# AWehenkel/Graphical-Normalizing-Flows

Measured on AMD Instinct MI355X. Metric: samples/sec (fwd+log|detJ|+bwd) MNIST d=784 Monotonic-DAG, higher is better.
Workload: dtype f32; 1 GPU; cfg4: MNIST d=784, MonotonicNormalizer[50,50,50] cond 30 S=20 + DAGConditioner(MNISTCNN->30, prior_A_kernel=2, hot_encoding=False, Gumbel gate T=1), b_size=100 per GPU; step = fwd+logdet+NLL+bwd+allreduce+Adam; global_batch=100, parallelism=dp1

## Files before the change

graphical-normalizing-flows_amd/gnf_hip/csrc/gnf_mnistcnn.h:

```cpp
#pragma once
#include "gnf_common.h"

namespace {

constexpr int IMG = 28, C1 = 26, C2 = 24, PO = 12, NCH = 16;
constexpr int ROWE = 36, ESZ = IMG * ROWE;
constexpr int ROW = 40, CH = C1 * ROW;
constexpr int ROWD = 40, CHD = 28 * ROWD + 16;
constexpr int CS = 676;
constexpr int NPOOL = NCH * PO * PO;
constexpr int FWD_WAVES = 8, BWD_WAVES = 8;
constexpr int PROW = NCH * 144 + NCH * 16 + NCH;

static_assert(CH % 32 == 16 && CHD % 32 == 16, "channel strides must sit 16 banks apart");

__device__ __forceinline__ f32x2 pk_v12(f32x2 a, f32x2 b) {
  f32x2 r;
  asm("v_pk_add_f32 %0, %1, %2 op_sel:[1,0] op_sel_hi:[1,0] neg_hi:[1,0]" : "=v"(r) : "v"(a), "v"(b));
  return r;
}
__device__ __forceinline__ void wino_in(const f32x2 (&lo)[4], const f32x2 (&hi)[4], float (&v)[16]) {
  f32x2 tl[4], th[4];
  tl[0] = lo[0] - lo[2]; th[0] = hi[0] - hi[2];
  tl[1] = lo[1] + lo[2]; th[1] = hi[1] + hi[2];
  tl[2] = lo[2] - lo[1]; th[2] = hi[2] - hi[1];
  tl[3] = lo[1] - lo[3]; th[3] = hi[1] - hi[3];
#pragma unroll
  for (int rr = 0; rr < 4; ++rr) {
    const f32x2 v03 = tl[rr] - th[rr], v12 = pk_v12(tl[rr], th[rr]);
    v[4 * rr + 0] = v03.x; v[4 * rr + 1] = v12.x; v[4 * rr + 2] = v12.y; v[4 * rr + 3] = v03.y;
  }
}

__device__ __forceinline__ float dpp_xor1(float v) {
  return __int_as_float(__builtin_amdgcn_update_dpp(0, __float_as_int(v), 0xB1, 0xF, 0xF, false));
}
__device__ __forceinline__ float dpp_xor8(float v) {
  return __int_as_float(__builtin_amdgcn_update_dpp(0, __float_as_int(v), 0x128, 0xF, 0xF, false));
}

struct CnnArgs {
  const float* e; const float* W1; const float* b1; const float* W2; const float* b2;
  float* pooled; unsigned char* arg;
  const float* gp; const unsigned char* argin; float* ge; float* part;
  int64_t n;
  const int32_t* plan; float* gec; int dplan;
};

template <int NU, int CHS>
__device__ __forceinline__ void conv1_units(const float* e_rd, float* a1_wr, int u0, const float* w1p, const f32x4& b1v,
                                            int q, int j, int lane) {
  u0 = __builtin_amdgcn_readfirstlane(u0);
  asm volatile("" : "+s"(u0));
  f32x16 acc[NU];
  float ev[NU][9], w1a[9];
#pragma unroll
  for (int tap = 0; tap < 9; ++tap) w1a[tap] = w1p[16 * tap];
#pragma unroll
  for (int k = 0; k < NU; ++k) {
    const int pos = 64 * (u0 + k) + lane;
    const int pc = pos < C1 * C1 ? pos : 0;
    const float* pe = e_rd + pc + 2 * (int)(__umul24((unsigned)pc, 2521u) >> 16);
#pragma unroll
    for (int tap = 0; tap < 9; ++tap) ev[k][tap] = pe[(tap / 3) * IMG + tap % 3];
#pragma unroll
    for (int v = 0; v < 16; ++v) acc[k][v] = b1v[v & 3];
  }
  __builtin_amdgcn_sched_barrier(0);
#pragma unroll
  for (int tap = 0; tap < 9; ++tap)
#pragma unroll
    for (int k = 0; k < NU; ++k) acc[k] = __builtin_amdgcn_mfma_f32_16x16x1f32(w1a[tap], ev[k][tap], acc[k], 0, 0, 0);
  __builtin_amdgcn_sched_barrier(0);
#pragma unroll
  for (int k = 0; k < NU; ++k)
#pragma unroll
    for (int b = 0; b < 4; ++b) {
      const int pos = 64 * (u0 + k) + 16 * b + j;
      if (pos < C1 * C1) {
        float* pa = a1_wr + 4 * q * CHS + pos + 2 * (int)(__umul24((unsigned)pos, 2521u) >> 16);
#pragma unroll
        for (int r = 0; r < 4; ++r) pa[r * CHS] = relu1(acc[k][4 * b + r]);
      }
    }
}
template <int CHS>
__device__ __forceinline__ void conv1_offsets(int u, int q, int j, int lane, unsigned (&po)[3]) {
  static_assert(CHS >= 26 * IMG + 8, "the dummy stores of off-grid positions land at 26 IMG + (0..7) of the channel");
  const int pos = 64 * u + lane, pc = pos < C1 * C1 ? pos : 0;
  unsigned w[4];
#pragma unroll
  for (int b = 0; b < 4; ++b) {
    const int p = 64 * u + 16 * b + j;
    w[b] = (unsigned)(4 * q * CHS + (p < C1 * C1 ? p + 2 * (p / C1) : 26 * IMG + (j & 7)));
  }
  po[0] = (unsigned)(pc + 2 * (pc / C1)) | (w[0] << 16);
  po[1] = w[1] | (w[2] << 16);
  po[2] = w[3];
}
template <int NU, int CHS>
__device__ __forceinline__ void conv1_units_pre(const float* e_rd, float* a1_wr, const unsigned (&po)[3][3], const float* w1p,
                                                const f32x4& b1v) {
  f32x16 acc[NU];
  float ev[NU][9], w1a[9];
#pragma unroll
  for (int tap = 0; tap < 9; ++tap) w1a[tap] = w1p[16 * tap];
#pragma unroll
  for (int k = 0; k < NU; ++k) {
    const float* pe = e_rd + (po[k][0] & 0xffffu);
#pragma unroll
    for (int tap = 0; tap < 9; ++tap) ev[k][tap] = pe[(tap / 3) * IMG + tap % 3];
#pragma unroll
    for (int v = 0; v < 16; ++v) acc[k][v] = b1v[v & 3];
  }
  __builtin_amdgcn_sched_barrier(0);
#pragma unroll
  for (int tap = 0; tap < 9; ++tap)
#pragma unroll
    for (int k = 0; k < NU; ++k) acc[k] = __builtin_amdgcn_mfma_f32_16x16x1f32(w1a[tap], ev[k][tap], acc[k], 0, 0, 0);
  __builtin_amdgcn_sched_barrier(0);
#pragma unroll
  for (int k = 0; k < NU; ++k) {
    const unsigned off[4] = {po[k][0] >> 16, po[k][1] & 0xffffu, po[k][1] >> 16, po[k][2]};
#pragma unroll
    for (int b = 0; b < 4; ++b) {
      float* pa = a1_wr + off[b];
#pragma unroll
// ... 38 lines not shown
```

graphical-normalizing-flows_amd/gnf_hip/csrc/gnf_mnistcnn.hip:

```cpp
#include "gnf_mnistcnn.h"

namespace {

#ifdef GNF_CNN_TIMING
#define TSTAMP(k) do { const long long t__ = __builtin_readcyclecounter(); tacc[k] += t__ - tlast; tlast = t__; } while (0)
#else
#define TSTAMP(k)
#endif

constexpr int NG4 = 11;
constexpr int USZ = 16 * 4 * 64;
constexpr int ROWB = 28, CHB = 730, A1B = NCH * CHB;
constexpr int ESZB = IMG * IMG;
constexpr int DCS = 648, DPAD = 576, DSZW = NCH * DCS;
static_assert(ROWB == IMG, "the de gather indexes the T planes with the pixel index");
static_assert(CHB >= 25 * ROWB + C1 && CHB % 4 == 2, "a1 channel stride");
static_assert(DCS % 64 == 8 && DCS >= DPAD + 64, "dY2 channel slots");
__device__ __forceinline__ int dslot(int o) { return (o & 3) + 4 * (o >> 3) + 8 * ((o >> 2) & 1); }

#ifndef GNF_BWD_C1U
#define GNF_BWD_C1U {0, 0, 0, 4, 1, 1, 2, 3}
#endif
__device__ constexpr int C1U[8] = GNF_BWD_C1U;
__device__ constexpr int C1PRO[8] = {2, 2, 2, 1, 1, 1, 1, 1};
constexpr int c1sum(const int (&a)[8]) { int s = 0; for (int i = 0; i < 8; ++i) s += a[i]; return s; }
constexpr int NU1 = (C1 * C1 + 63) / 64;
static_assert(c1sum(C1U) == NU1 && c1sum(C1PRO) == NU1, "conv1 units");

__device__ __forceinline__ void conv1_run(const float* e_rd, float* a1_wr, int u0, int nu, const float* w1a,
                                          const f32x4& b1v, int q, int j, int lane) {
  if (nu == 4) {
    conv1_units<2, CHB>(e_rd, a1_wr, u0, w1a, b1v, q, j, lane);
    conv1_units<2, CHB>(e_rd, a1_wr, u0 + 2, w1a, b1v, q, j, lane);
  } else if (nu == 3) conv1_units<3, CHB>(e_rd, a1_wr, u0, w1a, b1v, q, j, lane);
  else if (nu == 2) conv1_units<2, CHB>(e_rd, a1_wr, u0, w1a, b1v, q, j, lane);
  else if (nu == 1) conv1_units<1, CHB>(e_rd, a1_wr, u0, w1a, b1v, q, j, lane);
}

template <int HY>
__device__ __forceinline__ void dw2_phase(const float* av, const float* dz, f32x4 (&dU)[8]) {
  f32x4 zw[2];
  f32x2 dl[2][3], dh[2][3];
  auto load = [&](int st, int b) {
    const int tyl = st / 3, k = st - 3 * tyl;
    zw[b] = *reinterpret_cast<const f32x4*>(dz + 48 * tyl + 16 * k);
#pragma unroll
// ... 4 lines not shown
  };
  load(0, 0);
#pragma unroll
  for (int st = 0; st < 9; ++st) {
    const int b = st & 1;
    f32x2 tal, tah, tbl, tbh;
    float za[2], zb[2];
    if (HY == 0) {
      tal = dl[b][0] - dl[b][2]; tah = dh[b][0] - dh[b][2]; tbl = dl[b][1] + dl[b][2]; tbh = dh[b][1] + dh[b][2];
      za[0] = zw[b][0]; za[1] = zw[b][1]; zb[0] = zw[b][0] + zw[b][2]; zb[1] = zw[b][1] + zw[b][3];
    } else {
      tal = dl[b][1] - dl[b][0]; tah = dh[b][1] - dh[b][0]; tbl = dl[b][0] - dl[b][2]; tbh = dh[b][0] - dh[b][2];
      za[0] = zw[b][0] - zw[b][2]; za[1] = zw[b][1] - zw[b][3]; zb[0] = zw[b][2]; zb[1] = zw[b][3];
    }
    float vv[8], zz[8];
    {
      const f32x2 a03 = tal - tah, a12 = pk_v12(tal, tah), b03 = tbl - tbh, b12 = pk_v12(tbl, tbh);
      vv[0] = a03.x; vv[1] = a12.x; vv[2] = a12.y; vv[3] = a03.y;
      vv[4] = b03.x; vv[5] = b12.x; vv[6] = b12.y; vv[7] = b03.y;
    }
    zz[0] = za[0]; zz[1] = za[0] + za[1]; zz[2] = za[0] - za[1]; zz[3] = za[1];
    zz[4] = zb[0]; zz[5] = zb[0] + zb[1]; zz[6] = zb[0] - zb[1]; zz[7] = zb[1];
    if (st + 1 < 9) load(st + 1, b ^ 1);
    __builtin_amdgcn_sched_barrier(0);
#pragma unroll
    for (int xi = 0; xi < 8; ++xi) dU[xi] = mfma(zz[xi], vv[xi], dU[xi]);
    __builtin_amdgcn_sched_barrier(0);
  }
}

constexpr int KC = GNF_DAG_PLAN_KC;
template <bool SP>
__device__ __forceinline__ void cnn_bwd_body(const CnnArgs& a, float* smem) {
#ifdef GNF_CNN_TIMING
  long long tacc[8] = {0, 0, 0, 0, 0, 0, 0, 0};
  long long tlast = __builtin_readcyclecounter();
#endif
  float* e_s = smem;
  float* a1_s = smem + 2 * ESZB;
  float* d_s = a1_s + 2 * A1B;
  float* u_s = d_s + DSZW;
  unsigned* cnt_s = reinterpret_cast<unsigned*>(u_s + USZ);
  float* w1_s = u_s + USZ + 4;
  unsigned* gmt_s = reinterpret_cast<unsigned*>(w1_s + 9 * NCH);
  const int tid = threadIdx.x, lane = tid & 63, q = lane >> 4, j = lane & 15;
  const int wave = __builtin_amdgcn_readfirstlane(tid >> 6);
  constexpr int NW = BWD_WAVES, NT = 64 * BWD_WAVES;
  static_assert(((2 * ESZB) % 4 == 0) && ((2 * A1B) % 4 == 0) && (DSZW % 4 == 0), "d_s / u_s must be 16-B aligned");

  if (tid < 9 * NCH) w1_s[tid] = a.W1[(tid & 15) * 9 + (tid >> 4)];
  const float* w1a = w1_s + j;
  f32x4 b1v;
#pragma unroll
  for (int r = 0; r < 4; ++r) b1v[r] = a.b1[4 * q + r];
  float w1t[4];
#pragma unroll
  for (int r = 0; r < 4; ++r) w1t[r] = j < 9 ? a.W1[(4 * q + r) * 9 + j] : 0.f;

  if (wave < 4) {
    const int g = wave;
    const float* w = a.W2 + ((4 * q + g) * NCH + j) * 9;
    double gw[4][3];
#pragma unroll
    for (int c = 0; c < 3; ++c) {
      const double w0 = w[8 - c], w1 = w[5 - c], w2 = w[2 - c];
      gw[0][c] = w0; gw[1][c] = 0.5 * (w0 + w1 + w2); gw[2][c] = 0.5 * (w0 - w1 + w2); gw[3][c] = w2;
    }
#pragma unroll
    for (int r = 0; r < 4; ++r) {
      f32x4 u;
      u[0] = (float)gw[r][0];
      u[1] = (float)(0.5 * (gw[r][0] + gw[r][1] + gw[r][2]));
      u[2] = (float)(0.5 * (gw[r][0] - gw[r][1] + gw[r][2]));
      u[3] = (float)gw[r][2];
      *reinterpret_cast<f32x4*>(u_s + ((g * 4 + r) * 64 + lane) * 4) = u;
    }
  }

  const int hy = wave >> 2, wq = wave & 3;
  f32x4 dU[8];
#pragma unroll
  for (int xi = 0; xi < 8; ++xi) dU[xi] = f32x4{0.f, 0.f, 0.f, 0.f};
  f32x2 gW1p[2][10];
#pragma unroll
  for (int h = 0; h < 2; ++h)
#pragma unroll
    for (int k = 0; k < 10; ++k) gW1p[h][k] = f32x2{0.f, 0.f};
  float gb2 = 0.f;
  unsigned aprev = 0;

  for (int i = tid; i < DSZW; i += NT) d_s[i] = 0.f;
  for (int i = tid; i < 2 * A1B; i += NT) a1_s[i] = 0.f;
  if (tid == 0) *cnt_s = 0u;
  const int16_t* const pcols = SP ? reinterpret_cast<const int16_t*>(a.plan + a.dplan) : nullptr;
  if (SP) {
    for (int i = tid; i < a.dplan; i += NT) gmt_s[i] = 0u;
    __syncthreads();
    for (int t = tid; t < a.dplan * KC; t += NT) {
      const int jj = pcols[t];
      if (jj >= 0) {
        const int y = jj / IMG, x = jj - y * IMG;
        unsigned m = 0u;
#pragma unroll
        for (int ky = 0; ky < 3; ++ky)
#pragma unroll
          for (int kx = 0; kx < 3; ++kx) {
            const int py = y - ky, px = x - kx;
            if ((unsigned)py < (unsigned)C1 && (unsigned)px < (unsigned)C1) m |= 1u << ((13 * (py >> 1) + (px >> 1)) >> 4);
          }
        atomicOr(&gmt_s[t / KC], m);
      }
    }
  }

  constexpr int EPT = (IMG * IMG + NT - 1) / NT, WPT = (PO * PO + 31) / 32;
  float epre[EPT], gpre[WPT];
  unsigned apre[WPT];
  auto rsrc_of = [&](const void* base, int64_t im, int bytes) {
    return make_rsrc(static_cast<const char*>(base) + im * bytes, im < a.n ? bytes : 0);
  };
  const int vo_e = tid * 4, vo_g = ((tid >> 5) * (PO * PO) + (tid & 31)) * 4, vo_a = (tid >> 5) * (PO * PO) + (tid & 31);
  auto prefetch_e = [&](int64_t im) {
    const rsrc_t rs = rsrc_of(a.e, im, IMG * IMG * 4);
#pragma unroll
    for (int k = 0; k < EPT; ++k) epre[k] = __builtin_bit_cast(float, __builtin_amdgcn_raw_buffer_load_b32(rs, vo_e + k * NT * 4, 0, 0));
// ... 60 lines not shown
        const int y = (int)(__umul24((unsigned)ic, 2341u) >> 16);
        const float* tp = Tp + ic;
        float t[9];
#pragma unroll
        for (int tap = 0; tap < 9; ++tap) t[tap] = tp[tap * CHB - (tap / 3) * IMG - tap % 3];
        float s = 0.f;
#pragma unroll
        for (int ky = 0; ky < 3; ++ky) {
          const float r3 = (t[3 * ky] + t[3 * ky + 1]) + t[3 * ky + 2];
          s += (unsigned)(y - ky) < (unsigned)C1 ? r3 : 0.f;
        }
        __builtin_amdgcn_raw_buffer_store_b32(__builtin_bit_cast(unsigned, s), rs, i * 4, 0, 0);
      }
    }
  };

  auto de_cols = [&](int64_t im, int cj, const float* Tp) {
    const rsrc_t rs = rsrc_of(a.gec, im, KC * 4);
    const int ic = cj >= 0 ? cj : 0;
    const int y = (int)(__umul24((unsigned)ic, 2341u) >> 16);
    const float* tp = Tp + ic;
    float t[9];
#pragma unroll
    for (int tap = 0; tap < 9; ++tap) t[tap] = tp[tap * CHB - (tap / 3) * IMG - tap % 3];
    float sum = 0.f;
#pragma unroll
    for (int ky = 0; ky < 3; ++ky) {
      const float r3 = (t[3 * ky] + t[3 * ky + 1]) + t[3 * ky + 2];
      sum += (unsigned)(y - ky) < (unsigned)C1 ? r3 : 0.f;
    }
    __builtin_amdgcn_raw_buffer_store_b32(__builtin_bit_cast(unsigned, sum), rs, cj >= 0 && lane < KC ? lane * 4 : KC * 4, 0, 0);
  };

  const int64_t img0 = blockIdx.x, gstride = gridDim.x;
  const int rstep = SP ? (int)(gstride % a.dplan) : 0;
  int rowc = SP ? (int)(img0 % a.dplan) : 0, rowp = 0;
  prefetch_e(img0);
  prefetch_g(img0);
  stage_e(e_s);
  prefetch_e(img0 + gstride);
  __syncthreads();
  if (img0 < a.n) {
    int u0 = 0;
#pragma unroll
    for (int w = 0; w < NW; ++w) u0 += w < wave ? C1PRO[w] : 0;
    conv1_run(e_s, a1_s, u0, C1PRO[wave], w1a, b1v, q, j, lane);
  }

  auto scatter = [&]() {
    unsigned anew = 0;
#pragma unroll
    for (int k = 0; k < WPT; ++k)
      if ((tid & 31) + 32 * k < PO * PO) {
        const float g = gpre[k];
        const unsigned am = apre[k];
        gb2 += g;
        float* w = dwin + 128 * k;
        w[(aprev >> (2 * k)) & 3u] = 0.f;
        w[am] = g;
        anew |= am << (2 * k);
      }
    aprev = anew;
  };
  if (img0 < a.n) scatter();

  int par = 0;
  unsigned rd_target = 0;
  for (int64_t img = img0; img < a.n; img += gstride, par ^= 1) {
    float* a1p = a1_s + par * A1B;
    float* a1n = a1_s + (par ^ 1) * A1B;
    const float* e_rd = e_s + par * ESZB;
    float* e_nx = e_s + (par ^ 1) * ESZB;
    rd_target += NW;
    __syncthreads();
    TSTAMP(0);
    stage_e(e_nx);
    prefetch_e(img + 2 * gstride);
    prefetch_g(img + gstride);
    int cjp = -1;
    if (SP && wave == 0 && img != img0 && lane < KC) cjp = pcols[rowp * KC + lane];
    unsigned gm = 0x7FFu;
    if (SP) gm = __builtin_amdgcn_readfirstlane(gmt_s[rowc]);
    TSTAMP(1);
    if (hy == 0) dw2_phase<0>(a1p + vb, d_s + zb, dU);
    else dw2_phase<1>(a1p + vb, d_s + zb, dU);
    TSTAMP(2);
    if (SP) {
      if (wave == 0 && img != img0) de_cols(img - gstride, cjp, a1n);
    } else if (img != img0) de_gather(img - gstride, a1n);
#ifdef GNF_CNN_EXP_NOBMID
    if (!SP)
#endif
    __syncthreads();
    TSTAMP(3);
    const bool has_next = img + gstride < a.n;
    int c1t0 = 0;
#pragma unroll
    for (int w = 0; w < NW; ++w) c1t0 += w < wave ? C1U[w] : 0;
    const bool c1_first = wave != 7;
#ifdef GNF_CNN_EXP_NOCONV1
    const bool c1_on = false;
#else
    const bool c1_on = has_next;
#endif
    if (c1_on && c1_first) {
      conv1_run(e_nx, a1n, c1t0, C1U[wave], w1a, b1v, q, j, lane);
    }
    TSTAMP(4);
#pragma unroll
    for (int k = 0; k < 2; ++k) {
      const int grp = wave + NW * k;
      if (grp < NG4) {
        const unsigned tk = (tpk >> (16 * k)) & 0xFFFFu;
        const bool ok = tk != 0xFFFFu;
        const int to = ok ? (int)tk : 0;
        f32x4 m[16];
#pragma unroll
        for (int xi = 0; xi < 16; ++xi) m[xi] = f32x4{0.f, 0.f, 0.f, 0.f};
        const float* pwin[4];
#pragma unroll
        for (int wk = 0; wk < 4; ++wk) pwin[wk] = d_s + 4 * ((wpk[k][wk >> 1] >> (16 * (wk & 1))) & 0xFFFFu);
// ... 39 lines not shown
          dp[0][r] = (ok && g0.x > 0.f) ? y00 : 0.f;
          dp[1][r] = (ok && g0.y > 0.f) ? y01 : 0.f;
          dp[2][r] = (ok && g1.x > 0.f) ? y10 : 0.f;
          dp[3][r] = (ok && g1.y > 0.f) ? y11 : 0.f;
        }
        float ep[4][4];
        {
          const float* pe = e_rd + to;
#pragma unroll
          for (int rr = 0; rr < 4; ++rr) {
            const float2 lo = *reinterpret_cast<const float2*>(pe + rr * IMG);
            const float2 hi = *reinterpret_cast<const float2*>(pe + rr * IMG + 2);
            ep[rr][0] = lo.x; ep[rr][1] = lo.y; ep[rr][2] = hi.x; ep[rr][3] = hi.y;
          }
        }
#ifndef GNF_CNN_EXP_NODW1
#pragma unroll
        for (int h = 0; h < 2; ++h) {
          f32x2 d2[4];
#pragma unroll
          for (int p = 0; p < 4; ++p) d2[p] = f32x2{dp[p][2 * h], dp[p][2 * h + 1]};
          gW1p[h][9] += (d2[0] + d2[1]) + (d2[2] + d2[3]);
#pragma unroll
          for (int p = 0; p < 4; ++p) {
#pragma unroll
            for (int tap = 0; tap < 9; ++tap) {
              const float ev = ep[(p >> 1) + tap / 3][(p & 1) + tap % 3];
              gW1p[h][tap] = __builtin_elementwise_fma(d2[p], f32x2{ev, ev}, gW1p[h][tap]);
            }
            __builtin_amdgcn_sched_barrier(0);
          }
        }
#endif
        if (!SP || ((gm >> grp) & 1u)) {
          f32x4 tq[4];
#pragma unroll
          for (int p = 0; p < 4; ++p) tq[p] = f32x4{0.f, 0.f, 0.f, 0.f};
#pragma unroll
          for (int r = 0; r < 4; ++r)
#pragma unroll
            for (int p = 0; p < 4; ++p) tq[p] = mfma(w1t[r], dp[p][r], tq[p]);
#pragma unroll
          for (int r = 0; r < 4; ++r)
            if (ok && 4 * q + r < 9) {
              *reinterpret_cast<float2*>(pa + r * CHB) = make_float2(tq[0][r], tq[1][r]);
              *reinterpret_cast<float2*>(pa + r * CHB + ROWB) = make_float2(tq[2][r], tq[3][r]);
            }
        }
      }
      TSTAMP(5 + k);
    }
    if (c1_on && !c1_first) {
      conv1_run(e_nx, a1n, c1t0, C1U[wave], w1a, b1v, q, j, lane);
    }
    if (has_next) {
      while (__hip_atomic_load(cnt_s, __ATOMIC_ACQUIRE, __HIP_MEMORY_SCOPE_WORKGROUP) < rd_target) __builtin_amdgcn_s_sleep(1);
      scatter();
    }
    if (SP) { rowp = rowc; rowc += rstep; rowc -= rowc >= a.dplan ? a.dplan : 0; }
    TSTAMP(7);
  }
  __syncthreads();
  if (img0 < a.n) {
    const int64_t last = img0 + (a.n - 1 - img0) / gstride * gstride;
    if (SP) {
      if (wave == 0) de_cols(last, lane < KC ? (int)pcols[rowp * KC + lane] : -1, a1_s + (par ^ 1) * A1B);
    } else de_gather(last, a1_s + (par ^ 1) * A1B);
  }
#ifdef GNF_CNN_TIMING
  if (blockIdx.x == 7 && (tid & 63) == 0)
    for (int k = 0; k < 8; ++k) a.part[((int64_t)gridDim.x * NW + 1) * PROW + wave * 8 + k] = (float)tacc[k];
#endif

  __syncthreads();
  float* prow = smem + wave * PROW;
#pragma unroll
  for (int r = 0; r < 4; ++r) {
    dU[3][r] = -dU[3][r];
    if (hy == 0) dU[7][r] = -dU[7][r];
    else { dU[4][r] = -dU[4][r]; dU[5][r] = -dU[5][r]; dU[6][r] = -dU[6][r]; }
  }
#pragma unroll
  for (int r = 0; r < 4; ++r) {
    float ar[3][4];
#pragma unroll
    for (int x = 0; x < 4; ++x) {
      const float ua = dU[x][r], ub = dU[4 + x][r];
      if (hy == 0) { ar[0][x] = ua + 0.5f * ub; ar[1][x] = 0.5f * ub; ar[2][x] = 0.5f * ub; }
      else { ar[0][x] = 0.5f * ua; ar[1][x] = -0.5f * ua; ar[2][x] = 0.5f * ua + ub; }
    }
#pragma unroll
    for (int i = 0; i < 3; ++i) {
      float* o = prow + (4 * q + r) * 144 + j * 9 + 3 * i;
      o[0] = ar[i][0] + 0.5f * (ar[i][1] + ar[i][2]);
      o[1] = 0.5f * (ar[i][1] - ar[i][2]);
      o[2] = 0.5f * (ar[i][1] + ar[i][2]) + ar[i][3];
    }
  }
#pragma unroll
// ... 30 lines not shown
    cnn_bwd_body<true>(a, smem);
    return;
  }
  cnn_bwd_body<false>(a, smem);
}

__global__ __launch_bounds__(1024) void cnn_reduce_unpack_k(const float* __restrict__ part, int rows, float* gW1, float* gb1,
                                                            float* gW2, float* gb2) {
  __shared__ float red[16][64];
  const int lane = threadIdx.x & 63, wave = threadIdx.x >> 6;
  const int n = blockIdx.x * 64 + lane;
  float s0 = 0.f, s1 = 0.f;
  if (n < PROW) {
    const float* p = part + n;
    int r = wave;
    for (; r + 16 < rows; r += 32) { s0 += p[(int64_t)r * PROW]; s1 += p[(int64_t)(r + 16) * PROW]; }
    for (; r < rows; r += 16) s0 += p[(int64_t)r * PROW];
  }
  red[wave][lane] = s0 + s1;
  __syncthreads();
  if (wave != 0 || n >= PROW) return;
  float s = red[0][lane];
#pragma unroll
  for (int w = 1; w < 16; ++w) s += red[w][lane];
  if (n < NCH * 144) gW2[n] = s;
  else if (n < NCH * 144 + NCH * 16) {
    const int k = n - NCH * 144, oc = k >> 4, c = k & 15;
    if (c < 9) gW1[oc * 9 + c] = s;
    else if (c == 9) gb1[oc] = s;
  } else gb2[n - NCH * 144 - NCH * 16] = s;
}

constexpr int kPlanRows = IMG * IMG;
constexpr size_t kBwdWinoLds = (size_t)(2 * ESZB + 2 * A1B + DSZW + USZ + 4 + 9 * NCH + kPlanRows) * sizeof(float);
static_assert(kBwdWinoLds <= 160 * 1024, "conv backward LDS image");
static_assert((size_t)BWD_WAVES * PROW * sizeof(float) <= kBwdWinoLds, "the partial rows of the epilogue reuse the image LDS");
constexpr unsigned kBwdGrid = 256;

}

extern "C" {

int64_t gnf_mnistcnn_conv_bwd_ws_bytes(int64_t n_img) {
  (void)n_img;
  return ((int64_t)kBwdGrid * BWD_WAVES + 2) * PROW * (int64_t)sizeof(float);
}

int gnf_mnistcnn_conv_bwd(const float* e, const float* W1, const float* b1, const float* W2, const float* g_pooled,
                          const unsigned char* argmax, float* ge, float* gW1, float* gb1, float* gW2, float* gb2,
                          void* ws, int64_t ws_bytes, int64_t n_img, gnf_stream_t stream) {
  return gnf_mnistcnn_conv_bwd_cols(e, W1, b1, W2, g_pooled, argmax, ge, nullptr, 0, nullptr, gW1, gb1, gW2, gb2, ws,
                                    ws_bytes, n_img, stream);
}

int gnf_mnistcnn_conv_bwd_cols(const float* e, const float* W1, const float* b1, const float* W2, const float* g_pooled,
                               const unsigned char* argmax, float* ge, const int32_t* plan, int64_t d_plan,
                               float* ge_cols, float* gW1, float* gb1, float* gW2, float* gb2, void* ws,
                               int64_t ws_bytes, int64_t n_img, gnf_stream_t stream) {
  if (((!e || !g_pooled || !argmax || !ge) && n_img > 0) || !W1 || !b1 || !W2 || !gW1 || !gb1 || !gW2 || !gb2 || !ws ||
      n_img < 0)
    return GNF_EINVAL;
  if (plan && (!ge_cols && n_img > 0)) return GNF_EINVAL;
  if (plan && d_plan != kPlanRows) return GNF_ESHAPE;
  if (ws_bytes < gnf_mnistcnn_conv_bwd_ws_bytes(n_img)) return GNF_EWS;
  CnnArgs a{};
  a.e = e; a.W1 = W1; a.b1 = b1; a.W2 = W2; a.gp = g_pooled; a.argin = argmax; a.ge = ge; a.part = (float*)ws;
  a.n = n_img;
// ... 11 lines not shown
```

graphical-normalizing-flows_amd/gnf_hip/csrc/gnf_mnistcnn_fwd.hip:

```cpp
#include "gnf_mnistcnn.h"

namespace {

#ifdef GNF_CNN_TIMING
__device__ float g_fwd_timing[64];
__device__ long long g_fwd_start[1024];
#define TSTAMP(k) do { const long long t__ = __builtin_readcyclecounter(); tacc[k] += t__ - tlast; tlast = t__; } while (0)
#else
#define TSTAMP(k)
#endif

__global__ __launch_bounds__(64 * FWD_WAVES) void cnn_fwd_k(CnnArgs a) {
#ifdef GNF_CNN_TIMING
  long long tacc[8] = {0, 0, 0, 0, 0, 0, 0, 0};
  long long tlast = __builtin_readcyclecounter();
  const long long tstart0 = tlast;
#endif
  extern __shared__ __attribute__((aligned(16))) float smem[];
  float* e_s = smem;
  float* a1_s = smem + ESZ;
  const int tid = threadIdx.x, lane = tid & 63, q = lane >> 4, j = lane & 15;
  const int wave = __builtin_amdgcn_readfirstlane(tid >> 6);

  float w1f[3];
// ... 62 lines not shown
            accB = mfma(w2f[g * 9 + ky * 3 + kx], pB[o], accB);
          }
      }
#pragma unroll
      for (int half = 0; half < 2; ++half) {
        const f32x4 acc = half ? accB : accA;
        const int tt = half ? tB : t;
        if (half && tB == t) break;
#pragma unroll
        for (int r = 0; r < 4; ++r) {
          const float v00 = acc[r];
          const float v01 = dpp_xor1(v00), v10 = dpp_xor8(v00), v11 = dpp_xor8(v01);
          if ((j & 9) == 0) {
            float best = v00; int bi = 0;
            if (v01 > best) { best = v01; bi = 1; }
            if (v10 > best) { best = v10; bi = 2; }
            if (v11 > best) { best = v11; bi = 3; }
            const int64_t o = img * NPOOL + (4 * q + r) * (PO * PO) + (tt / 3) * PO + 4 * (tt % 3) + ((j & 7) >> 1);
            a.pooled[o] = best;
            a.arg[o] = (unsigned char)bi;
          }
        }
      }
    }
    TSTAMP(2);
  }
#ifdef GNF_CNN_TIMING
  if (blockIdx.x == 7 && (tid & 63) == 0)
    for (int k = 0; k < 3; ++k) g_fwd_timing[wave * 8 + k] = (float)tacc[k];
  if (tid == 0) { g_fwd_start[blockIdx.x] = tstart0; g_fwd_start[512 + blockIdx.x] = __builtin_readcyclecounter(); }
#endif
}

constexpr int WROW = IMG, WCH = 736, A1SZ = NCH * WCH, WESZ = IMG * IMG;
static_assert(WCH >= 25 * WROW + C1 && WCH % 64 == 32 && (2 * WROW - 22) % 32 == 2, "forward a1 layout");

#ifndef GNF_FWD_F1U
#define GNF_FWD_F1U {0, 0, 3, 2, 1, 1, 2, 2}
#endif
#ifndef GNF_FWD_SPLIT_WAVE
#define GNF_FWD_SPLIT_WAVE 0
#endif
__device__ constexpr int F1U[8] = GNF_FWD_F1U;
__device__ constexpr int F1PRO[8] = {2, 2, 2, 1, 1, 1, 1, 1};
constexpr int fsum(const int (&v)[8]) { int t = 0; for (int i = 0; i < 8; ++i) t += v[i]; return t; }
static_assert(fsum(F1U) == 11 && fsum(F1PRO) == 11, "conv1 units");
constexpr int fmax8(const int (&v)[8]) { int t = 0; for (int i = 0; i < 8; ++i) t = v[i] > t ? v[i] : t; return t; }
static_assert(fmax8(F1U) <= 3 && fmax8(F1PRO) <= 3, "at most three units per wavefront (conv1_do, the packed offsets)");

__global__ __launch_bounds__(64 * FWD_WAVES) void cnn_fwd_wino_k(CnnArgs a) {
  extern __shared__ __attribute__((aligned(16))) float smem[];
  float* e_s = smem;
  float* a1_s = smem + 2 * WESZ;
  float* xch = a1_s + 2 * A1SZ;
  float* w1_s = xch + 2 * 2 * 16 * 64;
  const int tid = threadIdx.x, lane = tid & 63, q = lane >> 4, j = lane & 15;
  const int wave = __builtin_amdgcn_readfirstlane(tid >> 6);
  constexpr int NW = FWD_WAVES, NT = 64 * FWD_WAVES;

  if (tid < 9 * NCH) w1_s[tid] = a.W1[(tid & 15) * 9 + (tid >> 4)];
  f32x4 b1v, b2v;
#pragma unroll
  for (int r = 0; r < 4; ++r) { b1v[r] = a.b1[4 * q + r]; b2v[r] = a.b2[4 * q + r]; }

  float uw[64];
#pragma unroll
  for (int g = 0; g < 4; ++g) {
    const float* w = a.W2 + (j * NCH + 4 * g + q) * 9;
    double gw[4][3];
#pragma unroll
    for (int c = 0; c < 3; ++c) {
      const double w0 = w[c], w1 = w[3 + c], w2 = w[6 + c];
      gw[0][c] = w0; gw[1][c] = 0.5 * (w0 + w1 + w2); gw[2][c] = 0.5 * (w0 - w1 + w2); gw[3][c] = w2;
    }
#pragma unroll
    for (int r = 0; r < 4; ++r) {
      uw[(4 * r + 0) * 4 + g] = (float)gw[r][0];
      uw[(4 * r + 1) * 4 + g] = (float)(0.5 * (gw[r][0] + gw[r][1] + gw[r][2]));
      uw[(4 * r + 2) * 4 + g] = (float)(0.5 * (gw[r][0] - gw[r][1] + gw[r][2]));
      uw[(4 * r + 3) * 4 + g] = (float)gw[r][2];
    }
  }

  auto rsrc_of = [&](const void* base, int64_t im, int bytes) {
    return make_rsrc(static_cast<const char*>(base) + im * bytes, im < a.n ? bytes : 0);
  };
  constexpr int EPT = (IMG * IMG + NT - 1) / NT;
  float pre[EPT];
  auto fetch = [&](int64_t im) {
    const rsrc_t rs = rsrc_of(a.e, im, IMG * IMG * 4);
#pragma unroll
    for (int k = 0; k < EPT; ++k) pre[k] = __builtin_bit_cast(float, __builtin_amdgcn_raw_buffer_load_b32(rs, (tid + k * NT) * 4, 0, 0));
  };
  auto stage = [&](float* dst) {
#pragma unroll
    for (int k = 0; k < EPT; ++k)
      if (tid + k * NT < IMG * IMG) dst[tid + k * NT] = pre[k];
  };
  auto half2 = [](const f32x4& v, int pr) { return pr ? f32x2{v[2], v[3]} : f32x2{v[0], v[1]}; };
  auto pool_out = [&](rsrc_t rp, rsrc_t ra, int t, int r, float v00, float v01, float v10, float v11) {
    float best = v00; int bi = 0;
    if (v01 > best) { best = v01; bi = 1; }
    if (v10 > best) { best = v10; bi = 2; }
    if (v11 > best) { best = v11; bi = 3; }
    const int o = (4 * q + r) * (PO * PO) + t;
    __builtin_amdgcn_raw_buffer_store_b32(__builtin_bit_cast(unsigned, best), rp, o * 4, 0, 0);
    __builtin_amdgcn_raw_buffer_store_b8((unsigned char)bi, ra, o, 0, 0);
  };
  auto finish_split = [&](const float* xb0, int64_t im) {
    const rsrc_t rp = rsrc_of(a.pooled, im, NPOOL * 4), ra = rsrc_of(a.arg, im, NPOOL);
    const float* xa = xb0 + lane;
#pragma unroll
    for (int r = 0; r < 4; ++r) {
      float v[4];
#pragma unroll
      for (int k = 0; k < 4; ++k) v[k] = xa[(r * 4 + k) * 64] + xa[16 * 64 + (r * 4 + k) * 64];
      pool_out(rp, ra, 16 * 8 + j, r, v[0], v[1], v[2], v[3]);
    }
  };
  auto conv1_do = [&](const float* e_rd, float* a1_wr, int u0, int nu) {
    if (nu == 3) conv1_units<3, WCH>(e_rd, a1_wr, u0, w1_s + j, b1v, q, j, lane);
    else if (nu == 2) conv1_units<2, WCH>(e_rd, a1_wr, u0, w1_s + j, b1v, q, j, lane);
    else if (nu == 1) conv1_units<1, WCH>(e_rd, a1_wr, u0, w1_s + j, b1v, q, j, lane);
  };
  auto whole_item = [&](const float* a1, int grp, int64_t im) {
    const int t = 16 * grp + j, ty = t / 12, tx = t - 12 * ty;
    const float* base = a1 + q * WCH + 2 * ty * WROW + 2 * tx;
    f32x4 acc[16];
#pragma unroll
    for (int xi = 0; xi < 16; ++xi) acc[xi] = f32x4{0.f, 0.f, 0.f, 0.f};
    acc[5] = b2v;
    f32x2 plo[4], phi[4];
#pragma unroll
    for (int rr = 0; rr < 4; ++rr) {
      plo[rr] = *reinterpret_cast<const f32x2*>(base + rr * WROW);
      phi[rr] = *reinterpret_cast<const f32x2*>(base + rr * WROW + 2);
    }
#pragma unroll
    for (int g = 0; g < 4; ++g) {
      float vv[16];
      wino_in(plo, phi, vv);
      if (g < 3) {
        const float* p = base + 4 * (g + 1) * WCH;
#pragma unroll
        for (int rr = 0; rr < 4; ++rr) {
          plo[rr] = *reinterpret_cast<const f32x2*>(p + rr * WROW);
          phi[rr] = *reinterpret_cast<const f32x2*>(p + rr * WROW + 2);
        }
      }
      __builtin_amdgcn_sched_barrier(0);
#pragma unroll
      for (int xi = 0; xi < 16; ++xi) acc[xi] = mfma(uw[xi * 4 + g], vv[xi], acc[xi]);
      __builtin_amdgcn_sched_barrier(0);
    }
    const rsrc_t rp = rsrc_of(a.pooled, im, NPOOL * 4), ra = rsrc_of(a.arg, im, NPOOL);
#pragma unroll
    for (int pr = 0; pr < 2; ++pr) {
      f32x2 s0[4], s1[4];
#pragma unroll
      for (int c = 0; c < 4; ++c) {
        const f32x2 m0 = half2(acc[c], pr), m1 = half2(acc[4 + c], pr), m2 = half2(acc[8 + c], pr), m3 = half2(acc[12 + c], pr);
        s0[c] = m0 + m1 + m2;
        s1[c] = m1 - m2 - m3;
      }
      const f32x2 y00 = s0[0] + s0[1] + s0[2], y01 = s0[1] - s0[2] - s0[3];
      const f32x2 y10 = s1[0] + s1[1] + s1[2], y11 = s1[1] - s1[2] - s1[3];
      pool_out(rp, ra, t, 2 * pr, y00.x, y01.x, y10.x, y11.x);
      pool_out(rp, ra, t, 2 * pr + 1, y00.y, y01.y, y10.y, y11.y);
    }
  };
  auto half_item = [&](const float* a1, int hf, float* xb0) {
    const int t = 16 * 8 + j, ty = t / 12, tx = t - 12 * ty;
    const float* base = a1 + q * WCH + 2 * ty * WROW + 2 * tx;
    f32x4 acc[8];
#pragma unroll
    for (int xi = 0; xi < 8; ++xi) acc[xi] = f32x4{0.f, 0.f, 0.f, 0.f};
    if (hf == 0) acc[5] = b2v;
    f32x2 plo[4], phi[4];
#pragma unroll
    for (int rr = 0; rr < 4; ++rr) {
      plo[rr] = *reinterpret_cast<const f32x2*>(base + rr * WROW);
      phi[rr] = *reinterpret_cast<const f32x2*>(base + rr * WROW + 2);
    }
#pragma unroll
    for (int g = 0; g < 4; ++g) {
      float vv[16];
      wino_in(plo, phi, vv);
      if (g < 3) {
        const float* p = base + 4 * (g + 1) * WCH;
#pragma unroll
        for (int rr = 0; rr < 4; ++rr) {
          plo[rr] = *reinterpret_cast<const f32x2*>(p + rr * WROW);
          phi[rr] = *reinterpret_cast<const f32x2*>(p + rr * WROW + 2);
        }
      }
      __builtin_amdgcn_sched_barrier(0);
      if (hf == 0) {
#pragma unroll
        for (int xi = 0; xi < 8; ++xi) acc[xi] = mfma(uw[xi * 4 + g], vv[xi], acc[xi]);
      } else {
#pragma unroll
        for (int xi = 0; xi < 8; ++xi) acc[xi] = mfma(uw[(8 + xi) * 4 + g], vv[8 + xi], acc[xi]);
      }
      __builtin_amdgcn_sched_barrier(0);
    }
    float* xb = xb0 + hf * 16 * 64 + lane;
#pragma unroll
    for (int pr = 0; pr < 2; ++pr) {
      f32x2 p0[4], p1[4];
#pragma unroll
      for (int c = 0; c < 4; ++c) {
        const f32x2 m0 = half2(acc[c], pr), m1 = half2(acc[4 + c], pr);
        p0[c] = hf == 0 ? m0 + m1 : m0;
        p1[c] = hf == 0 ? m1 : -m0 - m1;
      }
      const f32x2 y0 = p0[0] + p0[1] + p0[2], y1 = p0[1] - p0[2] - p0[3], y2 = p1[0] + p1[1] + p1[2], y3 = p1[1] - p1[2] - p1[3];
      xb[(2 * pr * 4 + 0) * 64] = y0.x; xb[(2 * pr * 4 + 1) * 64] = y1.x; xb[(2 * pr * 4 + 2) * 64] = y2.x; xb[(2 * pr * 4 + 3) * 64] = y3.x;
      xb[((2 * pr + 1) * 4 + 0) * 64] = y0.y; xb[((2 * pr + 1) * 4 + 1) * 64] = y1.y;
      xb[((2 * pr + 1) * 4 + 2) * 64] = y2.y; xb[((2 * pr + 1) * 4 + 3) * 64] = y3.y;
    }
  };

  const int64_t img0 = blockIdx.x, gs = gridDim.x;
  fetch(img0); stage(e_s);
  fetch(img0 + gs); stage(e_s + WESZ);
  fetch(img0 + 2 * gs);
  __syncthreads();
  {
    int u0 = 0;
#pragma unroll
    for (int w = 0; w < NW; ++w) u0 += w < wave ? F1PRO[w] : 0;
    if (img0 < a.n) conv1_do(e_s, a1_s, u0, F1PRO[wave]);
  }
  int c1u0 = 0;
#pragma unroll
  for (int w = 0; w < NW; ++w) c1u0 += w < wave ? F1U[w] : 0;
  unsigned upo[3][3];
#pragma unroll
  for (int k = 0; k < 3; ++k) conv1_offsets<WCH>(c1u0 + (k < F1U[wave] ? k : 0), q, j, lane, upo[k]);
  auto conv1_steady = [&](const float* e_rd, float* a1_wr) {
    const int nu = F1U[wave];
    if (nu == 3) conv1_units_pre<3, WCH>(e_rd, a1_wr, upo, w1_s + j, b1v);
    else if (nu == 2) conv1_units_pre<2, WCH>(e_rd, a1_wr, upo, w1_s + j, b1v);
    else if (nu == 1) conv1_units_pre<1, WCH>(e_rd, a1_wr, upo, w1_s + j, b1v);
  };
#ifndef GNF_FWD_UNITS_FIRST
#define GNF_FWD_UNITS_FIRST (wave >= 4)
#endif
  const bool units_first = GNF_FWD_UNITS_FIRST;

  int par = 0;
  int64_t prev = -1;
#ifdef GNF_CNN_TIMING
  long long tacc[8] = {0, 0, 0, 0, 0, 0, 0, 0};
  long long tlast = __builtin_readcyclecounter();
#define FSTAMP(k) do { const long long t__ = __builtin_readcyclecounter(); tacc[k] += t__ - tlast; tlast = t__; } while (0)
#else
#define FSTAMP(k)
#endif
  for (int64_t img = img0; img < a.n; img += gs, par ^= 1) {
    FSTAMP(5);
    __syncthreads();
    FSTAMP(0);
    const float* a1p = a1_s + par * A1SZ;
    float* a1n = a1_s + (par ^ 1) * A1SZ;
    const bool has_next = img + gs < a.n;
    stage(e_s + par * WESZ);
    fetch(img + 3 * gs);
    if (wave == GNF_FWD_SPLIT_WAVE && prev >= 0) finish_split(xch + (par ^ 1) * 2 * 16 * 64, prev);
    FSTAMP(1);
    if (has_next && units_first) conv1_steady(e_s + (par ^ 1) * WESZ, a1n);
    FSTAMP(2);
    whole_item(a1p, wave, img);
    FSTAMP(3);
    if (wave < 2) half_item(a1p, wave, xch + par * 2 * 16 * 64);
    FSTAMP(4);
    if (has_next && !units_first) conv1_steady(e_s + (par ^ 1) * WESZ, a1n);
    FSTAMP(2);
    prev = img;
  }
  __syncthreads();
  if (wave == GNF_FWD_SPLIT_WAVE && prev >= 0) finish_split(xch + (par ^ 1) * 2 * 16 * 64, prev);
#ifdef GNF_CNN_TIMING
  if (blockIdx.x == 7 && lane == 0)
    for (int k = 0; k < 8; ++k) a.pooled[wave * 8 + k] = (float)tacc[k];
#endif
#undef FSTAMP
}

constexpr size_t kFwdLds = (size_t)(ESZ + NCH * CH) * sizeof(float);
constexpr size_t kWinoLds = (size_t)(2 * WESZ + 2 * A1SZ + 2 * 2 * 16 * 64 + 9 * NCH) * sizeof(float);
static_assert(kWinoLds <= 160 * 1024, "one workgroup per CU");
constexpr unsigned kWinoGrid = 256;
constexpr unsigned kFwdGrid = 512;

}

extern "C" {

int gnf_mnistcnn_conv_fwd(const float* e, const float* W1, const float* b1, const float* W2, const float* b2,
                          float* pooled, unsigned char* argmax, int64_t n_img, int exact_ties, gnf_stream_t stream) {
  if (!W1 || !b1 || !W2 || !b2 || n_img < 0) return GNF_EINVAL;
  if (n_img == 0) return 0;
  if (!e || !pooled || !argmax) return GNF_EINVAL;
  CnnArgs a{};
  a.e = e; a.W1 = W1; a.b1 = b1; a.W2 = W2; a.b2 = b2; a.pooled = pooled; a.arg = argmax; a.n = n_img;
  if (exact_ties) {
    const unsigned grid = n_img < kFwdGrid ? (unsigned)n_img : kFwdGrid;
    return (int)gnf_launch_lds(cnn_fwd_k, dim3(grid), dim3(64 * FWD_WAVES), kFwdLds, (hipStream_t)stream, a);
  }
  const unsigned grid = n_img < kWinoGrid ? (unsigned)n_img : kWinoGrid;
  return (int)gnf_launch_lds(cnn_fwd_wino_k, dim3(grid), dim3(64 * FWD_WAVES), kWinoLds, (hipStream_t)stream, a);
}

}
```

Baseline: 17600 samples/s.

## Skew forward a1 channel groups, use packed subtracts, add direct backward de path

The forward conv1 output layout gets a 16-float skew between groups of four channels, so conv1 stores and Winograd patch reads from different groups land in different LDS banks. The Winograd output transforms now compute a-b-c with packed v_pk_add_f32 negation instead of scalar subtracts. The backward kernel gains an optional direct de_cols path, spread over four waves and gated behind GNF_BWD_DIRECT_DE, plus a small pad in front of the a1 buffer. The skew slightly enlarges LDS use and changes the offset packing, which now has to stay below 16 bits.

```diff
diff --git a/graphical-normalizing-flows_amd/gnf_hip/csrc/gnf_mnistcnn.h b/graphical-normalizing-flows_amd/gnf_hip/csrc/gnf_mnistcnn.h
--- a/graphical-normalizing-flows_amd/gnf_hip/csrc/gnf_mnistcnn.h
+++ b/graphical-normalizing-flows_amd/gnf_hip/csrc/gnf_mnistcnn.h
@@ -17,6 +17,11 @@
 __device__ __forceinline__ f32x2 pk_v12(f32x2 a, f32x2 b) {
   f32x2 r;
   asm("v_pk_add_f32 %0, %1, %2 op_sel:[1,0] op_sel_hi:[1,0] neg_hi:[1,0]" : "=v"(r) : "v"(a), "v"(b));
+  return r;
+}
+__device__ __forceinline__ f32x2 pk_sub(f32x2 a, f32x2 b) {
+  f32x2 r;
+  asm("v_pk_add_f32 %0, %1, %2 neg_lo:[0,1] neg_hi:[0,1]" : "=v"(r) : "v"(a), "v"(b));
   return r;
 }
 __device__ __forceinline__ void wino_in(const f32x2 (&lo)[4], const f32x2 (&hi)[4], float (&v)[16]) {
@@ -47,7 +52,7 @@
   const int32_t* plan; float* gec; int dplan;
 };
 
-template <int NU, int CHS>
+template <int NU, int CHS, int GS = 4 * CHS>
 __device__ __forceinline__ void conv1_units(const float* e_rd, float* a1_wr, int u0, const float* w1p, const f32x4& b1v,
                                             int q, int j, int lane) {
   u0 = __builtin_amdgcn_readfirstlane(u0);
@@ -78,21 +83,21 @@
     for (int b = 0; b < 4; ++b) {
       const int pos = 64 * (u0 + k) + 16 * b + j;
       if (pos < C1 * C1) {
-        float* pa = a1_wr + 4 * q * CHS + pos + 2 * (int)(__umul24((unsigned)pos, 2521u) >> 16);
+        float* pa = a1_wr + q * GS + pos + 2 * (int)(__umul24((unsigned)pos, 2521u) >> 16);
 #pragma unroll
         for (int r = 0; r < 4; ++r) pa[r * CHS] = relu1(acc[k][4 * b + r]);
       }
     }
 }
-template <int CHS>
+template <int CHS, int GS = 4 * CHS>
 __device__ __forceinline__ void conv1_offsets(int u, int q, int j, int lane, unsigned (&po)[3]) {
-  static_assert(CHS >= 26 * IMG + 8, "the dummy stores of off-grid positions land at 26 IMG + (0..7) of the channel");
+  static_assert(CHS >= 26 * IMG + 8 && 3 * GS + 4 * CHS < 65536, "the dummy stores of off-grid positions land at 26 IMG + (0..7) of the channel");
   const int pos = 64 * u + lane, pc = pos < C1 * C1 ? pos : 0;
   unsigned w[4];
 #pragma unroll
   for (int b = 0; b < 4; ++b) {
     const int p = 64 * u + 16 * b + j;
-    w[b] = (unsigned)(4 * q * CHS + (p < C1 * C1 ? p + 2 * (p / C1) : 26 * IMG + (j & 7)));
+    w[b] = (unsigned)(q * GS + (p < C1 * C1 ? p + 2 * (p / C1) : 26 * IMG + (j & 7)));
   }
   po[0] = (unsigned)(pc + 2 * (pc / C1)) | (w[0] << 16);
   po[1] = w[1] | (w[2] << 16);
diff --git a/graphical-normalizing-flows_amd/gnf_hip/csrc/gnf_mnistcnn.hip b/graphical-normalizing-flows_amd/gnf_hip/csrc/gnf_mnistcnn.hip
--- a/graphical-normalizing-flows_amd/gnf_hip/csrc/gnf_mnistcnn.hip
+++ b/graphical-normalizing-flows_amd/gnf_hip/csrc/gnf_mnistcnn.hip
@@ -12,6 +12,7 @@
 constexpr int USZ = 16 * 4 * 64;
 constexpr int ROWB = 28, CHB = 730, A1B = NCH * CHB;
 constexpr int ESZB = IMG * IMG;
+constexpr int A1PAD = 4;
 constexpr int DCS = 648, DPAD = 576, DSZW = NCH * DCS;
 static_assert(ROWB == IMG, "the de gather indexes the T planes with the pixel index");
 static_assert(CHB >= 25 * ROWB + C1 && CHB % 4 == 2, "a1 channel stride");
@@ -82,12 +83,17 @@
 constexpr int KC = GNF_DAG_PLAN_KC;
 template <bool SP>
 __device__ __forceinline__ void cnn_bwd_body(const CnnArgs& a, float* smem) {
+#ifdef GNF_BWD_DIRECT_DE
+  constexpr bool TP = !SP;
+#else
+  constexpr bool TP = true;
+#endif
 #ifdef GNF_CNN_TIMING
   long long tacc[8] = {0, 0, 0, 0, 0, 0, 0, 0};
   long long tlast = __builtin_readcyclecounter();
 #endif
   float* e_s = smem;
-  float* a1_s = smem + 2 * ESZB;
+  float* a1_s = smem + 2 * ESZB + A1PAD;
   float* d_s = a1_s + 2 * A1B;
   float* u_s = d_s + DSZW;
   unsigned* cnt_s = reinterpret_cast<unsigned*>(u_s + USZ);
@@ -96,7 +102,7 @@
   const int tid = threadIdx.x, lane = tid & 63, q = lane >> 4, j = lane & 15;
   const int wave = __builtin_amdgcn_readfirstlane(tid >> 6);
   constexpr int NW = BWD_WAVES, NT = 64 * BWD_WAVES;
-  static_assert(((2 * ESZB) % 4 == 0) && ((2 * A1B) % 4 == 0) && (DSZW % 4 == 0), "d_s / u_s must be 16-B aligned");
+  static_assert(((2 * ESZB + A1PAD) % 4 == 0) && ((2 * A1B) % 4 == 0) && (DSZW % 4 == 0), "d_s / u_s must be 16-B aligned");
 
   if (tid < 9 * NCH) w1_s[tid] = a.W1[(tid & 15) * 9 + (tid >> 4)];
   const float* w1a = w1_s + j;
@@ -105,7 +111,7 @@
   for (int r = 0; r < 4; ++r) b1v[r] = a.b1[4 * q + r];
   float w1t[4];
 #pragma unroll
-  for (int r = 0; r < 4; ++r) w1t[r] = j < 9 ? a.W1[(4 * q + r) * 9 + j] : 0.f;
+  for (int r = 0; r < 4; ++r) w1t[r] = (TP && j < 9) ? a.W1[(4 * q + r) * 9 + j] : 0.f;
 
   if (wave < 4) {
     const int g = wave;
@@ -140,7 +146,7 @@
   unsigned aprev = 0;
 
   for (int i = tid; i < DSZW; i += NT) d_s[i] = 0.f;
-  for (int i = tid; i < 2 * A1B; i += NT) a1_s[i] = 0.f;
+  for (int i = tid; i < A1PAD + 2 * A1B; i += NT) a1_s[i - A1PAD] = 0.f;
   if (tid == 0) *cnt_s = 0u;
   const int16_t* const pcols = SP ? reinterpret_cast<const int16_t*>(a.plan + a.dplan) : nullptr;
   if (SP) {
@@ -267,6 +273,39 @@
     __builtin_amdgcn_raw_buffer_store_b32(__builtin_bit_cast(unsigned, sum), rs, cj >= 0 && lane < KC ? lane * 4 : KC * 4, 0, 0);
   };
 
+  static_assert(KC == 32, "de_cols_direct: 8 passes of 4 column slots");
+  static_assert(2 * ESZB + A1PAD >= 2 * IMG + 2 && A1PAD >= 2, "de_cols_direct: reads in front of a1 buffer 0 stay inside LDS");
+  auto de_cols_direct = [&](int64_t im, int slot, int cj, const float* Dp) {
+    if (__builtin_amdgcn_ballot_w64(cj >= 0) == 0) return;
+    const rsrc_t rs = rsrc_of(a.gec, im, KC * 4);
+    const int tap = j < 9 ? j : 0, ky = tap / 3;
+    const int ic = cj >= 0 ? cj : 0;
+    const int y = (int)(__umul24((unsigned)ic, 2341u) >> 16);
+    const float* dp = Dp + ic - ky * IMG - (tap - 3 * ky);
+    f32x4 w[4];
+#pragma unroll
+    for (int k = 0; k < 4; ++k) w[k] = *reinterpret_cast<const f32x4*>(w1_s + 16 * tap + 4 * k);
+    float d[16];
+#pragma unroll
+    for (int c = 0; c < 16; ++c) d[c] = dp[c * CHB];
+    float t = 0.f;
+#pragma unroll
+    for (int r = 0; r < 4; ++r)
+#pragma unroll
+      for (int k = 0; k < 4; ++k) t = __builtin_fmaf(w[k][r], d[4 * k + r], t);
+    float r3 = (t + __shfl_down(t, 1, 16)) + __shfl_down(t, 2, 16);
+    r3 = (unsigned)(y - ky) < (unsigned)C1 ? r3 : 0.f;
+    float sum = 0.f + r3;
+    sum += __shfl_down(r3, 3, 16);
+    sum += __shfl_down(r3, 6, 16);
+    __builtin_amdgcn_raw_buffer_store_b32(__builtin_bit_cast(unsigned, sum), rs, cj >= 0 && j == 0 ? slot * 4 : KC * 4, 0, 0);
+  };
+  auto slot_of = [&](int k) { return 4 * (wave + 4 * k) + q; };
+  auto col_of = [&](int row, int k) -> int {
+    if (TP) return (k == 0 && wave == 0 && lane < KC) ? (int)pcols[row * KC + lane] : -1;
+    return wave < 4 ? (int)pcols[row * KC + slot_of(k)] : -1;
+  };
+
   const int64_t img0 = blockIdx.x, gstride = gridDim.x;
   const int rstep = SP ? (int)(gstride % a.dplan) : 0;
   int rowc = SP ? (int)(img0 % a.dplan) : 0, rowp = 0;
@@ -312,8 +351,8 @@
     stage_e(e_nx);
     prefetch_e(img + 2 * gstride);
     prefetch_g(img + gstride);
-    int cjp = -1;
-    if (SP && wave == 0 && img != img0 && lane < KC) cjp = pcols[rowp * KC + lane];
+    int cjp[2] = {-1, -1};
+    if (SP && img != img0) { cjp[0] = col_of(rowp, 0); cjp[1] = col_of(rowp, 1); }
     unsigned gm = 0x7FFu;
     if (SP) gm = __builtin_amdgcn_readfirstlane(gmt_s[rowc]);
     TSTAMP(1);
@@ -321,7 +360,11 @@
     else dw2_phase<1>(a1p + vb, d_s + zb, dU);
     TSTAMP(2);
     if (SP) {
-      if (wave == 0 && img != img0) de_cols(img - gstride, cjp, a1n);
+      if (TP) { if (wave == 0 && img != img0) de_cols(img - gstride, cjp[0], a1n); }
+      else if (wave < 4 && img != img0) {
+        de_cols_direct(img - gstride, slot_of(0), cjp[0], a1n);
+        de_cols_direct(img - gstride, slot_of(1), cjp[1], a1n);
+      }
     } else if (img != img0) de_gather(img - gstride, a1n);
 #ifdef GNF_CNN_EXP_NOBMID
     if (!SP)
@@ -427,7 +470,16 @@
           }
         }
 #endif
-        if (!SP || ((gm >> grp) & 1u)) {
+        if (!TP) {
+          if ((gm >> grp) & 1u) {
+#pragma unroll
+            for (int r = 0; r < 4; ++r)
+              if (ok) {
+                *reinterpret_cast<float2*>(pa + r * CHB) = make_float2(dp[0][r], dp[1][r]);
+                *reinterpret_cast<float2*>(pa + r * CHB + ROWB) = make_float2(dp[2][r], dp[3][r]);
+              }
+          }
+        } else if (!SP || ((gm >> grp) & 1u)) {
           f32x4 tq[4];
 #pragma unroll
           for (int p = 0; p < 4; ++p) tq[p] = f32x4{0.f, 0.f, 0.f, 0.f};
@@ -459,7 +511,11 @@
   if (img0 < a.n) {
     const int64_t last = img0 + (a.n - 1 - img0) / gstride * gstride;
     if (SP) {
-      if (wave == 0) de_cols(last, lane < KC ? (int)pcols[rowp * KC + lane] : -1, a1_s + (par ^ 1) * A1B);
+      if (TP) { if (wave == 0) de_cols(last, col_of(rowp, 0), a1_s + (par ^ 1) * A1B); }
+      else if (wave < 4) {
+        de_cols_direct(last, slot_of(0), col_of(rowp, 0), a1_s + (par ^ 1) * A1B);
+        de_cols_direct(last, slot_of(1), col_of(rowp, 1), a1_s + (par ^ 1) * A1B);
+      }
     } else de_gather(last, a1_s + (par ^ 1) * A1B);
   }
 #ifdef GNF_CNN_TIMING
@@ -556,7 +612,7 @@
 }
 
 constexpr int kPlanRows = IMG * IMG;
-constexpr size_t kBwdWinoLds = (size_t)(2 * ESZB + 2 * A1B + DSZW + USZ + 4 + 9 * NCH + kPlanRows) * sizeof(float);
+constexpr size_t kBwdWinoLds = (size_t)(2 * ESZB + A1PAD + 2 * A1B + DSZW + USZ + 4 + 9 * NCH + kPlanRows) * sizeof(float);
 static_assert(kBwdWinoLds <= 160 * 1024, "conv backward LDS image");
 static_assert((size_t)BWD_WAVES * PROW * sizeof(float) <= kBwdWinoLds, "the partial rows of the epilogue reuse the image LDS");
 constexpr unsigned kBwdGrid = 256;
diff --git a/graphical-normalizing-flows_amd/gnf_hip/csrc/gnf_mnistcnn_fwd.hip b/graphical-normalizing-flows_amd/gnf_hip/csrc/gnf_mnistcnn_fwd.hip
--- a/graphical-normalizing-flows_amd/gnf_hip/csrc/gnf_mnistcnn_fwd.hip
+++ b/graphical-normalizing-flows_amd/gnf_hip/csrc/gnf_mnistcnn_fwd.hip
@@ -118,8 +118,12 @@
 #endif
 }
 
-constexpr int WROW = IMG, WCH = 736, A1SZ = NCH * WCH, WESZ = IMG * IMG;
+#ifndef GNF_FWD_SKEW
+#define GNF_FWD_SKEW 16
+#endif
+constexpr int WROW = IMG, WCH = 736, WSK = GNF_FWD_SKEW, WG4 = 4 * WCH + WSK, A1SZ = 4 * WG4, WESZ = IMG * IMG;
 static_assert(WCH >= 25 * WROW + C1 && WCH % 64 == 32 && (2 * WROW - 22) % 32 == 2, "forward a1 layout");
+static_assert(WSK % 2 == 0 && (WSK == 0 || WG4 % 32 == 16), "group skew: 8-byte aligned patch reads, conv1 stores 16 banks apart");
 
 #ifndef GNF_FWD_F1U
 #define GNF_FWD_F1U {0, 0, 3, 2, 1, 1, 2, 2}
@@ -183,6 +187,11 @@
     for (int k = 0; k < EPT; ++k)
       if (tid + k * NT < IMG * IMG) dst[tid + k * NT] = pre[k];
   };
+#ifdef GNF_FWD_SCALAR_SUB
+#define FWD_SUB3(a, b, c) ((a) - (b) - (c))
+#else
+#define FWD_SUB3(a, b, c) pk_sub(pk_sub((a), (b)), (c))
+#endif
   auto half2 = [](const f32x4& v, int pr) { return pr ? f32x2{v[2], v[3]} : f32x2{v[0], v[1]}; };
   auto pool_out = [&](rsrc_t rp, rsrc_t ra, int t, int r, float v00, float v01, float v10, float v11) {
     float best = v00; int bi = 0;
@@ -205,9 +214,9 @@
     }
   };
   auto conv1_do = [&](const float* e_rd, float* a1_wr, int u0, int nu) {
-    if (nu == 3) conv1_units<3, WCH>(e_rd, a1_wr, u0, w1_s + j, b1v, q, j, lane);
-    else if (nu == 2) conv1_units<2, WCH>(e_rd, a1_wr, u0, w1_s + j, b1v, q, j, lane);
-    else if (nu == 1) conv1_units<1, WCH>(e_rd, a1_wr, u0, w1_s + j, b1v, q, j, lane);
+    if (nu == 3) conv1_units<3, WCH, WG4>(e_rd, a1_wr, u0, w1_s + j, b1v, q, j, lane);
+    else if (nu == 2) conv1_units<2, WCH, WG4>(e_rd, a1_wr, u0, w1_s + j, b1v, q, j, lane);
+    else if (nu == 1) conv1_units<1, WCH, WG4>(e_rd, a1_wr, u0, w1_s + j, b1v, q, j, lane);
   };
   auto whole_item = [&](const float* a1, int grp, int64_t im) {
     const int t = 16 * grp + j, ty = t / 12, tx = t - 12 * ty;
@@ -227,7 +236,7 @@
       float vv[16];
       wino_in(plo, phi, vv);
       if (g < 3) {
-        const float* p = base + 4 * (g + 1) * WCH;
+        const float* p = base + (g + 1) * WG4;
 #pragma unroll
         for (int rr = 0; rr < 4; ++rr) {
           plo[rr] = *reinterpret_cast<const f32x2*>(p + rr * WROW);
@@ -247,10 +256,10 @@
       for (int c = 0; c < 4; ++c) {
         const f32x2 m0 = half2(acc[c], pr), m1 = half2(acc[4 + c], pr), m2 = half2(acc[8 + c], pr), m3 = half2(acc[12 + c], pr);
         s0[c] = m0 + m1 + m2;
-        s1[c] = m1 - m2 - m3;
-      }
-      const f32x2 y00 = s0[0] + s0[1] + s0[2], y01 = s0[1] - s0[2] - s0[3];
-      const f32x2 y10 = s1[0] + s1[1] + s1[2], y11 = s1[1] - s1[2] - s1[3];
+        s1[c] = FWD_SUB3(m1, m2, m3);
+      }
+      const f32x2 y00 = s0[0] + s0[1] + s0[2], y01 = FWD_SUB3(s0[1], s0[2], s0[3]);
+      const f32x2 y10 = s1[0] + s1[1] + s1[2], y11 = FWD_SUB3(s1[1], s1[2], s1[3]);
       pool_out(rp, ra, t, 2 * pr, y00.x, y01.x, y10.x, y11.x);
       pool_out(rp, ra, t, 2 * pr + 1, y00.y, y01.y, y10.y, y11.y);
     }
@@ -273,7 +282,7 @@
       float vv[16];
       wino_in(plo, phi, vv);
       if (g < 3) {
-        const float* p = base + 4 * (g + 1) * WCH;
+        const float* p = base + (g + 1) * WG4;
 #pragma unroll
         for (int rr = 0; rr < 4; ++rr) {
           plo[rr] = *reinterpret_cast<const f32x2*>(p + rr * WROW);
@@ -300,7 +309,7 @@
         p0[c] = hf == 0 ? m0 + m1 : m0;
         p1[c] = hf == 0 ? m1 : -m0 - m1;
       }
-      const f32x2 y0 = p0[0] + p0[1] + p0[2], y1 = p0[1] - p0[2] - p0[3], y2 = p1[0] + p1[1] + p1[2], y3 = p1[1] - p1[2] - p1[3];
+      const f32x2 y0 = p0[0] + p0[1] + p0[2], y1 = FWD_SUB3(p0[1], p0[2], p0[3]), y2 = p1[0] + p1[1] + p1[2], y3 = FWD_SUB3(p1[1], p1[2], p1[3]);
       xb[(2 * pr * 4 + 0) * 64] = y0.x; xb[(2 * pr * 4 + 1) * 64] = y1.x; xb[(2 * pr * 4 + 2) * 64] = y2.x; xb[(2 * pr * 4 + 3) * 64] = y3.x;
       xb[((2 * pr + 1) * 4 + 0) * 64] = y0.y; xb[((2 * pr + 1) * 4 + 1) * 64] = y1.y;
       xb[((2 * pr + 1) * 4 + 2) * 64] = y2.y; xb[((2 * pr + 1) * 4 + 3) * 64] = y3.y;
@@ -323,7 +332,7 @@
   for (int w = 0; w < NW; ++w) c1u0 += w < wave ? F1U[w] : 0;
   unsigned upo[3][3];
 #pragma unroll
-  for (int k = 0; k < 3; ++k) conv1_offsets<WCH>(c1u0 + (k < F1U[wave] ? k : 0), q, j, lane, upo[k]);
+  for (int k = 0; k < 3; ++k) conv1_offsets<WCH, WG4>(c1u0 + (k < F1U[wave] ? k : 0), q, j, lane, upo[k]);
   auto conv1_steady = [&](const float* e_rd, float* a1_wr) {
     const int nu = F1U[wave];
     if (nu == 3) conv1_units_pre<3, WCH>(e_rd, a1_wr, upo, w1_s + j, b1v);
@@ -372,6 +381,7 @@
     for (int k = 0; k < 8; ++k) a.pooled[wave * 8 + k] = (float)tacc[k];
 #endif
 #undef FSTAMP
+#undef FWD_SUB3
 }
 
 constexpr size_t kFwdLds = (size_t)(ESZ + NCH * CH) * sizeof(float);
```

Result: no change. 17590 samples/s (-0.1%).
